# zeux/niagara

Measured on AMD Instinct MI355X. Metric: meshlets culled+compacted /sec, higher is better.
Workload: dtype f32; 1 GPU; config3A: 10000000 meshlets/GPU, 156250 task commands over 15625 draws, cone+frustum clustercull (LATE=0) + ordered compaction; meshlets_total=10000000, meshlets_rank0=10000000, commands_rank0=156250, draws_rank0=15625, streams=1, scatter_waves_per_workgroup=16, regime=one pass after the other on one stream, input_copies_rotated=4, count_reset=fused (NV_OPT_FUSED_COUNT_RESET), meshlet_layout=SoA12, visible_rank0=257819, visible_total=257819, counts_allreduce=none (N=1)

## Files before the change

niagara_amd/csrc/args.h:

```cpp
#pragma once

#include <hip/hip_runtime.h>
#include <stdint.h>

#include "../../include/niagara_vis.h"
#include "dealing.h"

#ifdef NV_EXPERIMENTS
#define NV_DBG(args, bits) (((args).debugMode & (bits)) != 0)
#else
#define NV_DBG(args, bits) false
#endif

namespace nv
{

#if defined(__HIP_DEVICE_COMPILE__) && !defined(__GFX9__)
#error "args.h: the DPP scans are written for GFX9-family wave64 targets (gfx950)"
#endif
#ifdef NV_EXPERIMENTS
#define NV_ASSERT_FULL_EXEC() do { if (__builtin_amdgcn_read_exec() != ~0ull) __builtin_trap(); } while (0)
#else
#define NV_ASSERT_FULL_EXEC() do { } while (0)
#endif

template <int CTRL, int ROW_MASK>
__device__ __forceinline__ uint32_t dpp_pull_u32(uint32_t v)
{
	return (uint32_t)__builtin_amdgcn_update_dpp(0, (int)v, CTRL, ROW_MASK, 0xf, false);
}

__device__ __forceinline__ uint32_t wave_scan_inclusive_u32(uint32_t v)
{
	NV_ASSERT_FULL_EXEC();
	v += dpp_pull_u32<0x111, 0xf>(v);
	v += dpp_pull_u32<0x112, 0xf>(v);
	v += dpp_pull_u32<0x114, 0xf>(v);
	v += dpp_pull_u32<0x118, 0xf>(v);
	v += dpp_pull_u32<0x142, 0xa>(v);
	v += dpp_pull_u32<0x143, 0xc>(v);
	return v;
}

template <int CTRL>
__device__ __forceinline__ uint32_t dpp_move_u32(uint32_t v)
{
	return (uint32_t)__builtin_amdgcn_update_dpp((int)v, (int)v, CTRL, 0xf, 0xf, false);
}
__device__ __forceinline__ uint32_t wave_shift_up1_u32(uint32_t v) { return dpp_move_u32<0x138>(v); }
__device__ __forceinline__ uint32_t quad_first_u32(uint32_t v) { return dpp_move_u32<0x00>(v); }
__device__ __forceinline__ uint32_t quad_xor1_u32(uint32_t v) { return dpp_move_u32<0xB1>(v); }
__device__ __forceinline__ uint32_t quad_xor2_u32(uint32_t v) { return dpp_move_u32<0x4E>(v); }

__device__ __forceinline__ uint32_t wave_sum_u32(uint32_t v)
{
	return (uint32_t)__builtin_amdgcn_readlane((int)wave_scan_inclusive_u32(v), 63);
}

constexpr uint32_t CC_MAX_SCATTER_TILES = 512;
constexpr uint32_t CC_COUNT_STRIDE = 16;
constexpr uint32_t CC_LISTS = 256;
struct ClusterCounts
{
	uint32_t parity;
	uint32_t k2parity;
	uint32_t base;
	uint32_t pad[29];
	uint32_t listOverflow[2];
	uint32_t pad2[30];
	uint32_t listCount[2][CC_LISTS * CC_COUNT_STRIDE];
	uint32_t counts[2][CC_MAX_SCATTER_TILES * CC_COUNT_STRIDE];
};

typedef __attribute__((address_space(4))) const uint32_t* nv_uniform_u32p;
__device__ __forceinline__ uint32_t load_uniform_u32(const uint32_t* p)
{
	return *(nv_uniform_u32p)(uintptr_t)p;
}

struct ClusterArgs
{
	NvCullData cd;
	NvPyramidDesc pyr;
	const NvMeshTaskCommand* __restrict__ commands;
	const uint32_t* __restrict__ count4;
	const NvMeshDraw* __restrict__ draws;
	const NvMeshlet* __restrict__ meshlets;
	const uint2* __restrict__ soaBounds;
	const uint32_t* __restrict__ soaCones;
	const float* __restrict__ poolBounds;
	const uint4* __restrict__ blockBounds;
	uint32_t blockMeshlets;
	uint32_t* __restrict__ mvb;
	uint32_t* __restrict__ clusterIndices;
	uint32_t* __restrict__ clusterCount4;
	uint32_t* __restrict__ payloadCounts;
	uint64_t* __restrict__ masks;
	uint4* __restrict__ candList;
	uint32_t listStride;
	uint32_t listMinPer;
	ClusterCounts* __restrict__ tileCounts;
	uint32_t scatterTiles;
	uint32_t generations;
	uint32_t dealScale;
	uint32_t cullWavesMagic;
	uint32_t genBlocks, genBlocksMagic;
	uint32_t tilesMagic;
	DealPlan plan;
	float filterK;
	float viewRowNorm;
	float viewTransNorm;
	float viewSum;
	uint32_t* hostHint;
	uint32_t commandCountOverride;
	float* __restrict__ probeOut;
#ifdef NV_EXPERIMENTS
	uint32_t debugMode;
#endif
	uint32_t fusedReset;
	uint32_t fusedSubmit;
	uint32_t deferHiz;
	uint32_t packBits;
	uint32_t packDirect;
	unsigned long long* countsSink;
};

struct DrawArgs
{
	NvCullData cd;
	NvPyramidDesc pyr;
	const NvMeshDraw* draws;
	const float4* __restrict__ soaWorld;
	const uint2* __restrict__ soaScaleMesh;
	const uint32_t* __restrict__ soaPostPass;
	const NvMesh* meshes;
	void* commands;
	uint32_t* count4;
	uint32_t* dvb;
	uint8_t* results;
	ClusterCounts* tileCounts;
	uint32_t scatterTiles;
	uint32_t fusedReset;
	uint32_t fusedSubmit;
	uint32_t meshCount;
	uint32_t* hostHint;
	uint32_t taskList;
	uint4* records;
	uint32_t* recordCounts;
	uint32_t recordsOn;
	uint32_t tileDraws;
	uint32_t unitsPerWave;
	uint32_t visFirst;
#ifdef NV_EXPERIMENTS
	uint32_t debugMode;
#endif
};

struct TriangleArgs
{
	NvGlobals globals;
	const NvMeshTaskCommand* __restrict__ commands;
	const NvMeshDraw* __restrict__ draws;
	const NvMeshlet* __restrict__ meshlets;
	const uint32_t* __restrict__ meshletData;
	const NvVertex* __restrict__ vertices;
	const uint32_t* __restrict__ clusterIndices;
	const uint32_t* __restrict__ cc4;
	NvTriangleMask* __restrict__ masks;
	uint32_t capacity;
	unsigned long long* __restrict__ totals;
	unsigned long long* __restrict__ partials;
};

struct RasterArgs
{
	NvGlobals globals;
	const NvMeshTaskCommand* __restrict__ commands;
	const NvMeshDraw* __restrict__ draws;
	const NvMeshlet* __restrict__ meshlets;
	const uint32_t* __restrict__ meshletData;
// ... 35 lines not shown
```

niagara_amd/csrc/clustercull.hip:

```cpp
#include <type_traits>

#include "cullmath.h"
#include "args.h"
#include "filtermath.h"
#include "dealing.h"
#include "cullform.h"

namespace nv
{

constexpr int CC_WAVES = 4;
constexpr int CC_THREADS = CC_WAVES * 64;


struct LaneData
{
	uint32_t b0, b1, cone;
	uint32_t mvbWord;
};

struct DrawUniform
{
	f3 q;
	float qw;
// ... 770 lines not shown
}

template <bool LATE, bool SOA, bool BITS, int CC_DA, bool DIRECT = false, bool DEFER = false, bool PACK = false>
__global__ __launch_bounds__(CC_THREADS, 6) void cluster_mask_kernel(ClusterArgs a)
{
	static_assert(!PACK || (DIRECT && SOA && !LATE), "the packed walk is a form of the direct early pass");
	const uint32_t lane = threadIdx.x & 63u;
	const uint32_t wave = __builtin_amdgcn_readfirstlane(threadIdx.x >> 6);
	const uint32_t w = blockIdx.x * CC_WAVES + wave;

	__shared__ float4 s_tab[PACK ? CC_WAVES : 1][PACK ? 64 : 1][CP_ENTRY / 16];
	__shared__ uint64_t s_heads[PACK ? CC_WAVES : 1][PACK ? CP_WINDOWS : 1];
	__shared__ uint64_t s_nout[PACK && !BITS ? CC_WAVES : 1][PACK && !BITS ? CP_WINDOWS : 1];

	__shared__ uint32_t s_mipTable[CC_WAVES][NV_MAX_MIPS];
	const uint32_t* s_mipOffset = s_mipTable[wave];
	if (LATE)
	{
		uint32_t off = 0;
#pragma unroll
		for (uint32_t i = 0; i < NV_MAX_MIPS; ++i)
			off = lane == i ? a.pyr.mipOffset[i] : off;
		if (lane < NV_MAX_MIPS)
			s_mipTable[wave][lane] = off;
	}

	if (!NV_DBG(a, 262144u))
		__builtin_amdgcn_s_setprio(3);
	const uint32_t gen = a.genBlocks ? div_launch_constant(blockIdx.x, a.genBlocks, a.genBlocksMagic) : 0u;
	float poolVmax3 = __builtin_inff(), poolRmax = __builtin_inff();
	uint32_t rawGroups, bankWord;
#ifdef NV_PLAIN_LOADS
	bankWord = load_uniform_u32(&a.tileCounts->parity);
	rawGroups = load_uniform_u32(a.count4 + 1);
	if (SOA)
	{
		k_f32p pb = (k_f32p)(uintptr_t)a.poolBounds;
		poolVmax3 = pb[0];
		poolRmax = pb[1];
	}
#else
	if (SOA)
	{
		uint64_t pool;
		asm volatile("s_nop 4\n\ts_load_dword %0, %3, 0x4\n\ts_load_dword %1, %4, 0x0\n\ts_load_dwordx2 %2, %5, 0x0\n\ts_waitcnt lgkmcnt(0)"
		             : "=&s"(rawGroups), "=&s"(bankWord), "=&s"(pool)
		             : "s"(a.count4), "s"(&a.tileCounts->parity), "s"(a.poolBounds)
		             : "memory");
		poolVmax3 = __uint_as_float((uint32_t)pool);
		poolRmax = __uint_as_float((uint32_t)(pool >> 32));
	}
	else
		asm volatile("s_nop 4\n\ts_load_dword %0, %2, 0x4\n\ts_load_dword %1, %3, 0x0\n\ts_waitcnt lgkmcnt(0)"
		             : "=&s"(rawGroups), "=&s"(bankWord)
		             : "s"(a.count4), "s"(&a.tileCounts->parity)
		             : "memory");
#endif
	const uint32_t numCmds = a.commandCountOverride ? a.commandCountOverride : (rawGroups < 65535u ? rawGroups : 65535u) * 64u;
	const uint32_t bank = bankWord & 1u;
	if (a.hostHint && blockIdx.x == 0 && threadIdx.x == 0)
		__hip_atomic_store(a.hostHint + (a.payloadCounts ? 4 : 0), numCmds, __ATOMIC_RELAXED, __HIP_MEMORY_SCOPE_SYSTEM);
	constexpr uint32_t CH = LATE ? CC_CHUNK_LATE : CC_CHUNK;
	const bool weightedWanted = !LATE && !NV_DBG(a, 32768u);
	const uint32_t planFlags = (weightedWanted ? DEAL_WEIGHTED_WANTED : 0u) | CH << 8;
	uint32_t chunkOf, myChunks, tileMul31, numTiles, gridWaves;
	bool dealtWeighted;
	{
		DealPlan plan;
		if (numCmds == a.plan.cmds && planFlags == a.plan.flags && !NV_DBG(a, 1073741824u))
			plan = a.plan;
		else
			plan = deal_plan(numCmds, CH, weightedWanted, gridDim.x * CC_WAVES, a.cullWavesMagic, a.generations, a.genBlocks, gridDim.x, a.dealScale, a.scatterTiles, a.tilesMagic);
		myChunks = deal_wave(plan, w, lane, gen, a.genBlocks * CC_WAVES, &chunkOf);
		gridWaves = plan.waves;
		dealtWeighted = plan.weighted != 0;
		tileMul31 = plan.tileMul31;
		numTiles = plan.numTiles;
	}
	const uint32_t myCmds = myChunks * CH;
	if (w == 0 && lane == 0)
	{
		a.tileCounts->k2parity = bank;
		a.tileCounts->base = a.fusedReset ? 0u : a.clusterCount4[0];
	}

	const bool dbgTime = NV_DBG(a, 8u) && a.probeOut;
	unsigned long long* stamps = reinterpret_cast<unsigned long long*>(a.probeOut) + (size_t)w * 8;
#define NV_STAMP(i) do { if (dbgTime && lane == 0) stamps[i] = __builtin_readcyclecounter(); } while (0)
	NV_STAMP(0);
	if (dbgTime && lane == 0)
		stamps[6] = wall_clock64();

	uint32_t passedFilter = 0;
#if defined(NV_FILLER_PS)
#pragma unroll
	for (int f = 0; f < NV_FILLER_PS; ++f)
		asm volatile("s_cmp_eq_u32 0, 0" : : : "scc");
#endif
#if defined(NV_FILLER_PV)
#pragma unroll
	for (int f = 0; f < NV_FILLER_PV; ++f)
		asm volatile("v_nop");
#endif
	for (uint32_t seg = 0; seg < myCmds; seg += 64)
	{
		const uint32_t cnt = myCmds - seg < 64u ? myCmds - seg : 64u;

		const uint32_t cidx = (seg + lane) / CH;
		const uint32_t chunk = dealtWeighted ? segment_chunk(chunkOf, seg >> 6) : cidx * gridWaves + w;
		const uint32_t myIdx = chunk * CH + (seg + lane) % CH;
		SegmentRegs r = {};
		if (lane < cnt && myIdx < numCmds)
		{
			const uint32_t* p = reinterpret_cast<const uint32_t*>(a.commands + myIdx);
			r.drawId = p[0];
			r.taskOffset = p[1];
			r.taskCount = p[2] < 64u ? p[2] : 64u;
			r.lateDrawVisibility = p[3];
			r.meshletVisibilityOffset = p[4];
		}
		if (!SOA)
		{
			if (r.taskCount)
			{
				const float4* d = reinterpret_cast<const float4*>(a.draws + r.drawId);
				r.d0 = d[0];
				r.d1 = d[1];
			}
			r.f = make_filter(a.cd, lane_draw(r), a.filterK, a.viewRowNorm, a.viewTransNorm, a.viewSum, poolVmax3, poolRmax);
		}
		NV_STAMP(1);

		constexpr bool FOLD_A = !LATE;
		constexpr bool BLOCK = SOA && !LATE && !BITS && !DIRECT && !DEFER;
		const bool foldSound = !FOLD_A || filter_fold_sound(a.cd.frustum);
		const bool useFilter = a.filterK > 0.0f && foldSound && !NV_DBG(a, 32u);
		u32x4 g0 = {}, g1 = {};
		auto gather_issue = [&]()
		{
			const char* dp = reinterpret_cast<const char*>(a.draws + (r.taskCount ? r.drawId : 0u));
#ifdef NV_PLAIN_LOADS
			g0 = reinterpret_cast<const u32x4*>(dp)[0];
			g1 = reinterpret_cast<const u32x4*>(dp)[1];
#else
			asm volatile("global_load_dwordx4 %0, %2, off\n\tglobal_load_dwordx4 %1, %2, off offset:16" : "=&v"(g0), "=&v"(g1) : "v"(dp) : "memory");
#endif
		};
		auto gather_finish = [&]()
		{
			r.d0 = make_float4(__uint_as_float(g0.x), __uint_as_float(g0.y), __uint_as_float(g0.z), __uint_as_float(g0.w));
			r.d1 = make_float4(__uint_as_float(g1.x), __uint_as_float(g1.y), __uint_as_float(g1.z), __uint_as_float(g1.w));
			r.f = make_filter<false>(a.cd, lane_draw(r), a.filterK, a.viewRowNorm, a.viewTransNorm, a.viewSum, poolVmax3, poolRmax);
			if (FOLD_A && !DIRECT)
			{
#pragma unroll
				for (int i = 0; i < 3; ++i)
				{
					r.fold[i] = a.cd.frustum[0] * r.f.m[i];
					r.fold[4 + i] = a.cd.frustum[2] * r.f.m[3 + i];
				}
				r.fold[3] = a.cd.frustum[0] * r.f.b[0];
				r.fold[7] = a.cd.frustum[2] * r.f.b[1];
			}
			if (!useFilter && !DIRECT)
				r.f.tK = __builtin_inff();
		};
// ... 467 lines not shown
			{
				const uint32_t n = (uint32_t)__builtin_popcountll(has);
				const uint32_t sub = w & (CC_LISTS - 1u);
				uint32_t slot = 0;
				if (lane == 0)
					slot = atomicAdd(&a.tileCounts->listCount[bank][sub * CC_COUNT_STRIDE], n);
				slot = __builtin_amdgcn_readfirstlane(slot);
				if (slot + n <= a.listStride)
				{
					if (has >> lane & 1ull)
					{
						uint4* e = a.candList + (size_t)(sub * a.listStride + slot + __builtin_amdgcn_mbcnt_hi((uint32_t)(has >> 32), __builtin_amdgcn_mbcnt_lo((uint32_t)has, 0u))) * 2u;
						e[0] = make_uint4(myIdx, r.drawId, r.taskOffset, r.taskCount);
						e[1] = make_uint4(r.lateDrawVisibility, r.meshletVisibilityOffset, maskLo, maskHi);
					}
				}
				else if (lane == 0)
					atomicOr(&a.tileCounts->listOverflow[bank], 1u);
			}
		}
		if (lane < cnt && myIdx < numCmds)
		{
			const uint64_t m = ((uint64_t)maskHi << 32) | maskLo;
			a.masks[myIdx] = m;
		}
		const bool payloadForm = !LATE && !DEFER && a.payloadCounts != nullptr;
		if (payloadForm)
		{
			const bool liveCmd = lane < cnt && myIdx < numCmds;
			const uint32_t mlo = liveCmd ? maskLo : 0u, mhi = liveCmd ? maskHi : 0u;
			if (liveCmd)
				a.payloadCounts[myIdx] = (uint32_t)__builtin_popcount(mlo) + (uint32_t)__builtin_popcount(mhi);
			for (uint64_t owners = __ballot((mlo | mhi) != 0); owners; owners &= owners - 1)
			{
				const uint32_t src = (uint32_t)__builtin_ctzll(owners);
				const uint32_t lo = __builtin_amdgcn_readlane(mlo, src), hi = __builtin_amdgcn_readlane(mhi, src);
				const uint32_t ci = __builtin_amdgcn_readlane(myIdx, src);
				if ((lane < 32u ? lo >> lane : hi >> (lane - 32u)) & 1u)
					a.clusterIndices[(size_t)ci * 64 + __builtin_amdgcn_mbcnt_hi(hi, __builtin_amdgcn_mbcnt_lo(lo, 0u))] = ci | (lane << 24);
			}
		}
		{
			const bool live = lane < cnt && myIdx < numCmds;
			const uint64_t m = live ? ((uint64_t)maskHi << 32) | maskLo : 0ull;
			const uint32_t tileOf = live ? deal_tile_of(myIdx, tileMul31) : ~0u;
			uint32_t pc = (uint32_t)__builtin_popcountll(m);
			const uint32_t tile0 = quad_first_u32(tileOf);
			const bool quadUniform = __all_quad_same(tileOf, tile0);
			if (quadUniform)
			{
				pc += quad_xor1_u32(pc);
				pc += quad_xor2_u32(pc);
				if (lane & 3u)
					pc = 0;
			}
			if (pc && !DEFER && !payloadForm && !NV_DBG(a, 2048u))
				atomicAdd(&a.tileCounts->counts[bank][tileOf * CC_COUNT_STRIDE], pc);
		}
	}
	if (lane == 0 && passedFilter && !(!LATE && !DEFER && a.payloadCounts != nullptr))
	{
		const uint32_t spread = numTiles ? (1u << (31 - __builtin_clz(numTiles))) - 1u : 0u;
		atomicAdd(&a.tileCounts->counts[bank][(w & spread) * CC_COUNT_STRIDE + 1], passedFilter);
	}
	NV_STAMP(5);
	if (dbgTime && lane == 0)
		stamps[7] = wall_clock64();
#undef NV_STAMP
}

template <int SC_WAVES>
__global__ __launch_bounds__(SC_WAVES * 64) void cluster_scatter_kernel(ClusterArgs a)
{
	constexpr uint32_t SC_THREADS = SC_WAVES * 64;
	__shared__ uint32_t s_part[SC_WAVES];
	__shared__ uint32_t s_sum[SC_WAVES];
	constexpr uint32_t STEP = 1024, PER_LANE = STEP / SC_THREADS;
	constexpr int TILE_LOADS = (int)((CC_MAX_SCATTER_TILES + SC_THREADS - 1) / SC_THREADS);

	const uint32_t tid = threadIdx.x;
	const uint32_t lane = tid & 63u;
	const uint32_t wave = __builtin_amdgcn_readfirstlane(tid >> 6);

	const uint32_t numCmds = indirect_command_count(a);
	const uint32_t T = scatter_tile_commands(numCmds, a.scatterTiles, a.tilesMagic);
	const uint32_t numTiles = (numCmds + T - 1) / T;
	const uint32_t tile = blockIdx.x;
	const bool dbgNoScatter = NV_DBG(a, 4u);

	const uint32_t k2parity = load_uniform_u32(&a.tileCounts->k2parity);
	const uint32_t base0 = load_uniform_u32(&a.tileCounts->base);
	uint32_t cnt0[TILE_LOADS] = {}, cnt1[TILE_LOADS] = {};
	uint32_t pf0[TILE_LOADS] = {}, pf1[TILE_LOADS] = {};
#pragma unroll
	for (int j = 0; j < TILE_LOADS; ++j)
	{
		const uint32_t i = j * SC_THREADS + tid;
		if (i < numTiles)
		{
			cnt0[j] = a.tileCounts->counts[0][i * CC_COUNT_STRIDE];
			cnt1[j] = a.tileCounts->counts[1][i * CC_COUNT_STRIDE];
			pf0[j] = a.tileCounts->counts[0][i * CC_COUNT_STRIDE + 1];
			pf1[j] = a.tileCounts->counts[1][i * CC_COUNT_STRIDE + 1];
		}
	}
	const uint32_t first = tile * T;
	const uint32_t n = tile < numTiles ? (numCmds - first < T ? numCmds - first : T) : 0u;
	uint64_t m4[PER_LANE];
	if (PER_LANE == 4)
	{
		const uint32_t c = tid * PER_LANE;
		const ulonglong2* src = reinterpret_cast<const ulonglong2*>(a.masks + first + c);
		ulonglong2 lo = make_ulonglong2(0, 0), hi = make_ulonglong2(0, 0);
		if (c < n)
		{
			lo = src[0];
			hi = src[1];
		}
		m4[0] = c + 0 < n ? lo.x : 0ull;
		m4[PER_LANE > 1 ? 1 : 0] = c + 1 < n ? lo.y : 0ull;
		m4[PER_LANE > 2 ? 2 : 0] = c + 2 < n ? hi.x : 0ull;
		m4[PER_LANE > 3 ? 3 : 0] = c + 3 < n ? hi.y : 0ull;
	}
	else
	{
#pragma unroll
		for (uint32_t j = 0; j < PER_LANE; ++j)
			m4[j] = tid * PER_LANE + j < n ? a.masks[first + tid * PER_LANE + j] : 0ull;
	}

	const uint32_t bank = k2parity & 1u;
	for (uint32_t i = tile * SC_THREADS + tid; i < CC_MAX_SCATTER_TILES; i += gridDim.x * SC_THREADS)
	{
		a.tileCounts->counts[bank ^ 1u][i * CC_COUNT_STRIDE] = 0;
		a.tileCounts->counts[bank ^ 1u][i * CC_COUNT_STRIDE + 1] = 0;
		if (i < CC_LISTS)
			a.tileCounts->listCount[bank ^ 1u][i * CC_COUNT_STRIDE] = 0;
	}
	if (tile == 0 && tid == 0)
	{
		a.tileCounts->parity = bank ^ 1u;
		a.tileCounts->listOverflow[bank ^ 1u] = 0;
		if (numTiles == 0 && a.hostHint)
			__hip_atomic_store(a.hostHint + 1, 0u, __ATOMIC_RELAXED, __HIP_MEMORY_SCOPE_SYSTEM);
		if (numTiles == 0)
		{
			if (a.fusedReset)
				a.clusterCount4[0] = 0;
			if (a.countsSink)
			{
				a.countsSink[0] = 0;
				a.countsSink[1] = a.count4[0];
				a.countsSink[2] = a.fusedReset ? 0u : a.clusterCount4[0];
			}
			if (a.fusedSubmit)
			{
				const uint32_t raw = a.fusedReset ? 0u : a.clusterCount4[0];
				const uint32_t count = raw < NV_CLUSTER_LIMIT ? raw : NV_CLUSTER_LIMIT;
				const uint32_t gy = (count + 255u) / 256u;
				a.clusterCount4[1] = NV_CLUSTER_TILE;
				a.clusterCount4[2] = gy < 65535u ? gy : 65535u;
				a.clusterCount4[3] = 256u / NV_CLUSTER_TILE;
				for (uint32_t i = count; i < ((count + 255u) & ~255u); ++i)
					a.clusterIndices[i] = ~0u;
			}
		}
	}
	if (tile >= numTiles)
		return;

	uint32_t before = 0, all = 0, passed = 0;
#pragma unroll
	for (int j = 0; j < TILE_LOADS; ++j)
	{
		const uint32_t i = j * SC_THREADS + tid;
		const uint32_t v = bank ? cnt1[j] : cnt0[j];
		all += v;
		before += i < tile ? v : 0u;
		passed += bank ? pf1[j] : pf0[j];
	}
	if (tile == numTiles - 1 && a.hostHint)
	{
		__shared__ uint32_t s_passed;
		if (tid == 0)
			s_passed = 0;
		__syncthreads();
		const uint32_t wp = wave_sum_u32(passed);
		if (lane == 0 && wp)
			atomicAdd(&s_passed, wp);
		__syncthreads();
		if (tid == 0)
			__hip_atomic_store(a.hostHint + 1, s_passed, __ATOMIC_RELAXED, __HIP_MEMORY_SCOPE_SYSTEM);
	}
	const uint32_t wBefore = wave_sum_u32(before), wAll = wave_sum_u32(all);
	if (lane == 0)
	{
		s_part[wave] = wBefore;
		s_sum[wave] = wAll;
	}
	__syncthreads();
	uint32_t running = base0, total = base0;
#pragma unroll
	for (int w = 0; w < SC_WAVES; ++w)
	{
		running += s_part[w];
		total += s_sum[w];
	}
	if (tid == 0 && tile == numTiles - 1)
	{
		a.clusterCount4[0] = total;
		if (a.countsSink)
		{
			a.countsSink[0] = 0;
			a.countsSink[1] = a.count4[0];
			a.countsSink[2] = total;
		}
	}
	if (a.fusedSubmit && tile == numTiles - 1)
	{
		const uint32_t count = total < NV_CLUSTER_LIMIT ? total : NV_CLUSTER_LIMIT;
		if (tid == 0)
		{
			const uint32_t gy = (count + 255u) / 256u;
			a.clusterCount4[1] = NV_CLUSTER_TILE;
			a.clusterCount4[2] = gy < 65535u ? gy : 65535u;
			a.clusterCount4[3] = 256u / NV_CLUSTER_TILE;
		}
		const uint32_t boundary = (count + 255u) & ~255u;
		if (count + tid < boundary)
			a.clusterIndices[count + tid] = ~0u;
	}

	for (uint32_t c0 = 0; c0 < n; c0 += STEP)
	{
		if (c0)
		{
			const uint32_t c = c0 + tid * PER_LANE;
#pragma unroll
			for (uint32_t j = 0; j < PER_LANE; ++j)
				m4[j] = c + j < n ? a.masks[first + c + j] : 0ull;
		}
		uint32_t pc[PER_LANE], mine = 0;
#pragma unroll
		for (uint32_t j = 0; j < PER_LANE; ++j)
		{
			pc[j] = (uint32_t)__builtin_popcountll(m4[j]);
			mine += pc[j];
		}
		uint32_t incl = wave_scan_inclusive_u32(mine);
		__syncthreads();
		if (lane == 63)
			s_part[wave] = incl;
		__syncthreads();
		uint32_t excl = running + incl - mine;
#pragma unroll
		for (int w = 0; w < SC_WAVES; ++w)
		{
			uint32_t p = s_part[w];
			excl += w < (int)wave ? p : 0u;
			running += p;
		}

		const bool mayOverflow = running > NV_CLUSTER_LIMIT;
		auto emit = [&](auto checked)
		{
#pragma unroll
			for (uint32_t j = 0; j < PER_LANE; ++j)
			{
				uint64_t owners = dbgNoScatter ? 0ull : __ballot(pc[j] != 0);
				while (owners)
				{
					const int src = __builtin_ctzll(owners);
					asm("s_bitset0_b64 %0, %1" : "+s"(owners) : "s"(src));
					const uint32_t mlo = __builtin_amdgcn_readlane((uint32_t)m4[j], src);
					const uint32_t mhi = __builtin_amdgcn_readlane((uint32_t)(m4[j] >> 32), src);
					const uint32_t off = __builtin_amdgcn_readlane(excl, src);
					const uint64_t ms = ((uint64_t)mhi << 32) | mlo;
					if (ms >> lane & 1ull)
					{
						uint32_t rank = __builtin_amdgcn_mbcnt_hi(mhi, __builtin_amdgcn_mbcnt_lo(mlo, 0u));
						uint32_t index = off + rank;
						if (!decltype(checked)::value || index < NV_CLUSTER_LIMIT)
							a.clusterIndices[index] = (first + c0 + (wave * 64 + src) * PER_LANE + j) | (lane << 24);
					}
				}
				excl += pc[j];
			}
		};
		if (mayOverflow)
			emit(std::true_type{});
		else
			emit(std::false_type{});
	}
}

constexpr int CH_THREADS = 256;
constexpr int CH_CMDS = 128;
#ifndef NV_CH_U
#define NV_CH_U 4
#endif
constexpr int CH_U = NV_CH_U;

#define NV_LDS_BARRIER() asm volatile("s_waitcnt lgkmcnt(0)\n\ts_barrier" ::: "memory")

struct HizTimes
{
	bool on;
	uint64_t prev;
	uint64_t acc[6];
	uint32_t rounds;
};
#ifdef NV_EXPERIMENTS
#define NV_HIZ_T(T, i, drain)                                                  \
	do                                                                         \
	{                                                                          \
		if ((T).on)                                                            \
		{                                                                      \
			if (drain)                                                         \
				asm volatile("s_waitcnt vmcnt(0) lgkmcnt(0)" ::: "memory");    \
			const uint64_t now = __builtin_readcyclecounter();                 \
			(T).acc[i] += now - (T).prev;                                      \
			(T).prev = now;                                                    \
		}                                                                      \
	} while (0)
#else
#define NV_HIZ_T(T, i, drain) do { } while (0)
#endif

template <int U, bool SOA, bool FIRST>
NV_DEV void hiz_round(const ClusterArgs& a, uint32_t base, uint32_t total, uint32_t tid, bool ownsDraw, const float4& d0, const float4& d1,
                      const uint16_t* s_list, const uint32_t* s_taskOffset, float4 (*s_draw)[2], const MipRecord* s_mip, uint32_t* s_visLo, uint32_t* s_visHi,
                      HizTimes& T)
{
	const float* __restrict__ texels = a.pyr.d_base;
	uint32_t e[U];
	uint2 b[U];
#pragma unroll
	for (int k = 0; k < U; ++k)
	{
		const uint32_t s = base + k * CH_THREADS + tid;
		e[k] = s_list[s < total ? s : total - 1u];
		const uint32_t mi = s_taskOffset[e[k] >> 6] + (e[k] & 63u);
		if (SOA)
			b[k] = a.soaBounds[mi];
		else
			b[k] = *reinterpret_cast<const uint2*>(a.meshlets + mi);
	}
	if (FIRST)
	{
		if (ownsDraw)
		{
			s_draw[tid][0] = d0;
			s_draw[tid][1] = d1;
		}
		NV_LDS_BARRIER();
	}
	NV_HIZ_T(T, 1, true);
	float depth[U];
	uint32_t use[U];
	float t00[U], t10[U], t01[U], t11[U];
#pragma unroll
	for (int k = 0; k < U; ++k)
	{
		const float4 q0 = s_draw[e[k] >> 6][0], q1 = s_draw[e[k] >> 6][1];
		DrawUniform u;
		u.pos = { q0.x, q0.y, q0.z };
		u.scale = q0.w;
		u.q = { q1.x, q1.y, q1.z };
		u.qw = q1.w;
		LaneData l;
		l.b0 = b[k].x;
		l.b1 = b[k].y;
		l.cone = 0;
		l.mvbWord = 0;
		f3 c;
// ... 356 lines not shown
			const float len = __builtin_amdgcn_sqrtf(__builtin_fmaf(cx, cx, __builtin_fmaf(cy, cy, cz * cz)));
			const float rhs = __builtin_fmaf(kc * 0.00787401574803149606f, len, scale * rad);
			const float D = lhs - rhs;
			const bool cull = D > Tc, keep = D < -Tc;
			decided = decided && (out || cull || keep);
			visible = visible && keep;
		}
		if (!decided && !NV_DBG(a, 536870912u))
		{
			const float4 q0 = s_draw[owner][0], q1 = s_draw[owner][1];
			DrawUniform u;
			u.pos = { q0.x, q0.y, q0.z };
			u.scale = q0.w;
			u.q = { q1.x, q1.y, q1.z };
			u.qw = q1.w;
			LaneData l;
			l.b0 = b0;
			l.b1 = b1;
			l.cone = cone[k];
			l.mvbWord = 0;
			f3 c;
			float r;
			lane_sphere(cd, u, l, c, r);
			visible = frustum_test(cd, c, r);
			if (cd.clusterBackfaceEnabled != 0 && visible)
			{
				f3 axis;
				float cutoff;
				lane_cone(cd, u, l, axis, cutoff);
				visible = !cone_cull(c, r, axis, cutoff);
			}
		}
		if (STAT)
		{
			const bool passes = s < total && !(useCert && out);
			const uint64_t passM = __ballot(passes);
			const uint32_t lane = tid & 63u;
			const uint32_t prevOwner = wave_shift_up1_u32(owner);
			if (passes && (lane == 0u || prevOwner != owner || !(passM >> (lane - 1u) & 1ull)))
				s_passed[owner] = 1u;
		}
		if (s < total && !visible)
			atomicAnd(bit < 32u ? &s_visLo[owner] : &s_visHi[owner], ~(1u << (bit & 31u)));
	}
}

struct BitsCommand
{
	uint32_t drawId, taskOffset, taskCount, mvo;
};

NV_DEV BitsCommand bits_load_command(const ClusterArgs& a, uint32_t idx, bool live)
{
	const uint32_t* p = reinterpret_cast<const uint32_t*>(a.commands + (live ? idx : 0u));
	BitsCommand c;
	c.drawId = p[0];
	c.taskOffset = p[1];
	c.taskCount = p[2] < 64u ? p[2] : 64u;
	c.mvo = p[4];
	return c;
}

template <bool SOA, bool BITS>
__global__ __launch_bounds__(CB_THREADS, 4) void cluster_bits_kernel(ClusterArgs a)
{
	__shared__ uint32_t s_visLo[CB_CMDS], s_visHi[CB_CMDS], s_taskOffset[CB_CMDS], s_excl[CB_CMDS], s_passed[BITS ? 1 : CB_CMDS];
	__shared__ float4 s_draw[CB_CMDS][2];
	__shared__ float4 s_cert[CB_CMDS][5];
	__shared__ uint16_t s_list[CB_CMDS * 64];
	__shared__ uint32_t s_part[CB_THREADS / 64];

	const uint32_t tid = threadIdx.x;
	const uint32_t lane = tid & 63u;
	const uint32_t wave = __builtin_amdgcn_readfirstlane(tid >> 6);
	const uint32_t numCmds = indirect_command_count(a);
	if (a.hostHint && blockIdx.x == 0 && tid == 0)
		__hip_atomic_store(a.hostHint + (a.payloadCounts ? 4 : 0), numCmds, __ATOMIC_RELAXED, __HIP_MEMORY_SCOPE_SYSTEM);
	const uint32_t T2 = scatter_tile_commands(numCmds, a.scatterTiles, a.tilesMagic);
	const uint32_t bank = load_uniform_u32(&a.tileCounts->parity) & 1u;
	if (blockIdx.x == 0 && tid == 0)
	{
		a.tileCounts->k2parity = bank;
		a.tileCounts->base = a.fusedReset ? 0u : a.clusterCount4[0];
	}
	if (numCmds == 0)
		return;
	const uint32_t G = gridDim.x;
	const uint32_t iters = (numCmds + G * (uint32_t)CB_CMDS - 1u) / (G * (uint32_t)CB_CMDS);
	uint32_t per = iters ? (numCmds + G * iters - 1u) / (G * iters) : 0u;
	per = per < 16u ? 16u : per;
	uint32_t passedAcc = 0;

	uint32_t chunk = blockIdx.x;
	BitsCommand cur = bits_load_command(a, chunk * per + tid, tid < per && chunk * per + tid < numCmds);
	BitsCommand nxt = bits_load_command(a, (chunk + G) * per + tid, tid < per && (chunk + G) * per + tid < numCmds);
	float4 d0, d1;
	uint32_t oldw[3];
	auto load_dependents = [&](const BitsCommand& c, bool liveC, float4& o0, float4& o1, uint32_t* w)
	{
		const uint32_t tc = liveC ? c.taskCount : 0u;
		const float4* dp = reinterpret_cast<const float4*>(a.draws + (tc ? c.drawId : 0u));
		o0 = dp[0];
		o1 = dp[1];
		const uint32_t w0 = tc ? c.mvo >> 5 : 0u, wLast = tc ? (c.mvo + tc - 1u) >> 5 : 0u;
#pragma unroll
		for (uint32_t j = 0; j < 3; ++j)
			w[j] = BITS ? a.mvb[w0 + j < wLast ? w0 + j : wLast] : 0u;
	};
	load_dependents(cur, tid < per && chunk * per + tid < numCmds, d0, d1, oldw);
	asm volatile("; prologue loads landed" : "+v"(d0.x), "+v"(d0.y), "+v"(d0.z), "+v"(d0.w), "+v"(d1.x), "+v"(d1.y), "+v"(d1.z), "+v"(d1.w), "+v"(oldw[0]), "+v"(oldw[1]), "+v"(oldw[2]),
	             "+v"(nxt.drawId), "+v"(nxt.taskOffset), "+v"(nxt.taskCount), "+v"(nxt.mvo));

	for (; chunk * per < numCmds; chunk += G)
	{
		const uint32_t idx = chunk * per + tid;
		const bool live = tid < per && idx < numCmds;
		const uint32_t taskCount = live ? cur.taskCount : 0u;
		uint64_t cand = 0;
		{
			const uint32_t sh = cur.mvo & 31u;
			uint64_t old = 0;
#pragma unroll
			for (int j = 0; j < 3; ++j)
			{
				const int lo = 32 * j - (int)sh;
				if (lo >= (int)taskCount)
					break;
				old |= lo >= 0 ? (uint64_t)oldw[j] << lo : (uint64_t)(oldw[j] >> (-lo));
			}
			const uint64_t valid = taskCount >= 64u ? ~0ull : (1ull << taskCount) - 1ull;
			cand = BITS ? old & valid : valid;
		}

		const uint32_t pc = (uint32_t)__builtin_popcountll(cand);
		uint32_t incl = wave_scan_inclusive_u32(pc);
		if (lane == 63)
			s_part[wave] = incl;
		if (tid < CB_CMDS)
		{
			s_visLo[tid] = (uint32_t)cand;
			s_visHi[tid] = (uint32_t)(cand >> 32);
			s_taskOffset[tid] = cur.taskOffset;
			s_excl[tid] = incl - pc;
			if (!BITS)
				s_passed[tid] = 0u;
		}

		const float4 c0 = d0, c1 = d1;
		float4 n0, n1;
		uint32_t neww[3];
		load_dependents(nxt, tid < per && idx + G * per < numCmds, n0, n1, neww);
		const uint32_t idx2 = (chunk + 2u * G) * per + tid;
		const BitsCommand nn = bits_load_command(a, idx2, tid < per && idx2 < numCmds);
		NV_LDS_BARRIER();

		uint32_t total = 0;
		{
			const uint32_t p0 = s_part[0], p1 = s_part[1];
			total = p0 + p1;
			if (NV_DBG(a, 67108864u))
			{
				uint32_t at = tid < (uint32_t)CB_CMDS ? s_excl[tid] + (tid >= 64u ? p0 : 0u) : 0u;
				for (uint64_t rest = cand; rest; rest &= rest - 1)
					s_list[at++] = (uint16_t)((tid << 6) | (uint32_t)__builtin_ctzll(rest));
			}
			else
// ... 364 lines not shown
```

niagara_amd/csrc/context.hip:

```cpp
#include <hip/hip_runtime.h>

#include <atomic>
#include <new>
#include <algorithm>
#include <vector>
#include <stdlib.h>
#include <stdint.h>
#include <string.h>
#include <math.h>

#include "../../include/niagara_vis.h"
#include "cullmath.h"
#include "args.h"
#include "filtermath.h"
#include "cullform.h"

namespace nv
{

int launch_cluster_mask(hipStream_t, const ClusterArgs&, const CullForm&, uint32_t maskBlocks);
int launch_cluster_scatter(hipStream_t, const ClusterArgs&, uint32_t scatterBlocks, uint32_t waves);
int launch_cluster_hiz(hipStream_t, const ClusterArgs&, bool soa, uint32_t gridBlocks);
int launch_cluster_bits(hipStream_t, const ClusterArgs&, bool soa, uint32_t gridBlocks);
size_t clustercull_mask_bytes();
// ... 804 lines not shown

	if (nv::drawcull_result_bytes(cull->drawCount) > ctx->drawResultsCapacity)
		return NV_ENOMEM;
	int rc = NV_OK;

	nv::DrawArgs a;
	a.cd = *cull;
	a.pyr = pyramid ? *pyramid : null_pyramid();
	a.draws = d_draws;
	const size_t drawOffset = ctx->scene->drawsFrom && d_draws >= ctx->scene->drawsFrom ? (size_t)(d_draws - ctx->scene->drawsFrom) : ~size_t(0);
	const bool mirrored = ctx->scene->soaWorld && drawOffset != ~size_t(0) && ctx->scene->drawsFrom + drawOffset == d_draws &&
	                      drawOffset + cull->drawCount <= ctx->scene->drawsCount && ctx->scene->drawsMeshes == d_meshes;
	a.soaWorld = mirrored ? ctx->scene->soaWorld + drawOffset : nullptr;
	a.soaScaleMesh = mirrored ? ctx->scene->soaScaleMesh + drawOffset : nullptr;
	a.soaPostPass = mirrored ? ctx->scene->soaPostPass + drawOffset : nullptr;
	a.meshes = d_meshes;
	a.commands = d_commands;
	a.count4 = d_count4;
	a.dvb = d_drawVisibility;
	a.results = ctx->drawResults;
	a.tileCounts = ctx->drawTileCounts;
	a.scatterTiles = scatter_grid(ctx);
#ifdef NV_EXPERIMENTS
	a.debugMode = ctx->debugMode;
#endif
	a.fusedReset = ctx->fusedReset;
	a.fusedSubmit = ctx->fusedSubmit;
	a.meshCount = ctx->scene->meshesFrom == d_meshes ? ctx->scene->meshCount : 0u;
	a.hostHint = ctx->hintDevice;
	a.taskList = ctx->forceTaskList >= 0 ? (uint32_t)ctx->forceTaskList : (ctx->hintHost && ctx->hintHost[3] > 4u * ctx->hintHost[2] ? 1u : 0u);
	a.visFirst = late ? 0u : (ctx->forceVisFirst >= 0 ? (uint32_t)ctx->forceVisFirst : (ctx->hintHost && ctx->hintHost[2] != 0u && (uint64_t)ctx->hintHost[2] * 8u < cull->drawCount ? 1u : 0u));
	if (task)
	{
		ctx->variants[a.taskList ? NV_VARIANT_TASK_LIST : NV_VARIANT_TASK_PER_DRAW] += 1u;
		ctx->taskCommandsFrom = d_commands;
	}
	hipEvent_t e0 = prof_mark(ctx, (hipStream_t)stream);
	rc = nv::launch_drawcull((hipStream_t)stream, a, late, task);
	prof_push(ctx, NV_PROF_DRAWCULL, e0, prof_mark(ctx, (hipStream_t)stream));
	return rc;
}

int nv_reset_count(nv_context* ctx, void* stream, uint32_t* d_count4a, uint32_t* d_count4b)
{
	if (!ctx || (!d_count4a && !d_count4b))
		return NV_EINVAL;
	DeviceGuard guard(ctx->device);
	return nv::launch_reset_count((hipStream_t)stream, d_count4a, d_count4b);
}

int nv_tasksubmit(nv_context* ctx, void* stream, uint32_t* d_count4, NvMeshTaskCommand* d_commands)
{
	if (!ctx || !d_count4 || !d_commands)
		return NV_EINVAL;
	DeviceGuard guard(ctx->device);
	return nv::launch_tasksubmit((hipStream_t)stream, d_count4, d_commands);
}

static int fill_cluster_args(nv_context* ctx, nv::ClusterArgs& a, const NvCullData* cull, int late,
                             const NvMeshTaskCommand* d_commands, const uint32_t* d_count4, const NvMeshDraw* d_draws,
                             const NvMeshlet* d_meshlets, uint32_t* d_meshletVisibility, const NvPyramidDesc* pyramid)
{
	if (!ctx || !cull || !d_commands || !d_draws || !d_meshlets)
		return NV_EINVAL;
	if (cull->clusterOcclusionEnabled == 1 && !d_meshletVisibility)
		return NV_EINVAL;
	if (late && cull->clusterOcclusionEnabled == 1 && !(pyramid && pyramid->d_base))
		return NV_EINVAL;
	memset(&a, 0, sizeof(a));
	a.cd = *cull;
	a.pyr = pyramid ? *pyramid : null_pyramid();
	a.commands = d_commands;
	a.count4 = d_count4;
	a.draws = d_draws;
	a.meshlets = d_meshlets;
	const bool soa = ctx->scene->mirroredFrom == d_meshlets && ctx->scene->soaBounds && ctx->scene->poolWords;
	a.soaBounds = soa ? ctx->scene->soaBounds : nullptr;
	a.soaCones = soa ? ctx->scene->soaCones : nullptr;
	a.poolBounds = soa ? reinterpret_cast<const float*>(ctx->scene->poolWords + 2) : nullptr;
	a.blockBounds = soa ? ctx->scene->blockBounds : nullptr;
	a.blockMeshlets = soa ? ctx->scene->mirroredCount : 0u;
	a.mvb = d_meshletVisibility;
	a.masks = ctx->masks;
	a.candList = ctx->candList;
	a.listStride = ctx->listStride;
	a.listMinPer = ctx->listMinPer;
	a.tileCounts = ctx->tileCounts;
	a.scatterTiles = scatter_grid(ctx);
	a.generations = ctx->ccBlocksPerCU;
	a.dealScale = ctx->dealScale;
	{
		const uint32_t cullGrid = persistent_grid(ctx, ctx->ccBlocksPerCU);
		a.cullWavesMagic = nv_division_magic(cullGrid * 4u);
		a.genBlocks = cullGrid / 6u ? cullGrid / 6u : 1u;
		a.genBlocksMagic = nv_division_magic(a.genBlocks);
		a.tilesMagic = nv_division_magic(a.scatterTiles);
	}
	a.filterK = nv::filter_k(cull->frustum, cull->znear, cull->zfar);
	nv::filter_view_norms(cull->view, &a.viewRowNorm, &a.viewTransNorm, &a.viewSum);
	a.hostHint = ctx->hintDevice;
	return NV_OK;
}

int nv_clustercull(nv_context* ctx, void* stream, const NvCullData* cull, int late, const NvMeshTaskCommand* d_commands,
                   const uint32_t* d_count4, const NvMeshDraw* d_draws, const NvMeshlet* d_meshlets,
                   uint32_t* d_meshletVisibility, const NvPyramidDesc* pyramid, uint32_t* d_clusterIndices,
                   uint32_t* d_clusterCount4)
{
	if (!d_count4 || !d_clusterIndices || !d_clusterCount4)
		return NV_EINVAL;
	nv::ClusterArgs a;
	int rc = fill_cluster_args(ctx, a, cull, late, d_commands, d_count4, d_draws, d_meshlets, d_meshletVisibility, pyramid);
	if (rc)
		return rc;
	DeviceGuard guard(ctx->device);
	a.clusterIndices = d_clusterIndices;
	a.clusterCount4 = d_clusterCount4;
	a.fusedReset = ctx->fusedReset;
	a.fusedSubmit = ctx->fusedSubmit;
	a.countsSink = reinterpret_cast<unsigned long long*>(ctx->countsSink);
#ifdef NV_EXPERIMENTS
	a.debugMode = ctx->debugMode;
	if (ctx->debugMode & (8u | 268435456u))
	{
		const size_t timingWaves = std::max((size_t)persistent_grid(ctx, 8) * 4, (size_t)ctx->listSharers * nv::CC_LISTS * 4);
		if (ctx->timing && ctx->timingWaves < timingWaves)
		{
			scratch_free(ctx->timing);
			ctx->timing = nullptr;
		}
		if (!ctx->timing && scratch_alloc(&ctx->timing, timingWaves * 8 * sizeof(unsigned long long)) == hipSuccess)
			ctx->timingWaves = timingWaves;
		a.probeOut = ctx->timing;
	}
#endif
	hipStream_t s = (hipStream_t)stream;
	hipEvent_t e0 = prof_mark(ctx, s);
	const bool twoStage = launch_cull(ctx, s, a, false, late, d_commands, &rc).twoStage;
	ctx->variants[NV_VARIANT_HIZ_STAGE] += twoStage ? 1u : 0u;
	hipEvent_t e1 = prof_mark(ctx, s);
	hipEvent_t eh = e1;
	if (rc == 0 && twoStage)
	{
		const uint32_t blocks = ctx->listSharers * nv::CC_LISTS;
		rc = nv::launch_cluster_hiz(s, a, a.soaBounds != nullptr, blocks);
		eh = prof_mark(ctx, s);
	}
	if (rc == 0 && !(ctx->debugMode & 16u))
		rc = nv::launch_cluster_scatter(s, a, a.scatterTiles, ctx->scatterWaves);
	hipEvent_t e2 = prof_mark(ctx, s);
	prof_push(ctx, NV_PROF_CLUSTER_CULL, e0, e1);
	if (twoStage)
		prof_push(ctx, NV_PROF_CLUSTER_HIZ, e1 ? e1 : nullptr, eh);
	prof_push(ctx, NV_PROF_CLUSTER_SCATTER, eh ? eh : nullptr, e2);
	return rc;
}

int nv_clustersubmit(nv_context* ctx, void* stream, uint32_t* d_clusterCount4, uint32_t* d_clusterIndices)
{
	if (!ctx || !d_clusterCount4 || !d_clusterIndices)
		return NV_EINVAL;
	DeviceGuard guard(ctx->device);
	return nv::launch_clustersubmit((hipStream_t)stream, d_clusterCount4, d_clusterIndices);
}

int nv_taskcull(nv_context* ctx, void* stream, const NvCullData* cull, int late, const NvMeshTaskCommand* d_commands,
                const uint32_t* d_count4, const NvMeshDraw* d_draws, const NvMeshlet* d_meshlets,
                uint32_t* d_meshletVisibility, const NvPyramidDesc* pyramid, uint32_t* d_payloads, uint32_t* d_payloadCounts)
{
	if (!d_count4 || !d_payloads || !d_payloadCounts)
		return NV_EINVAL;
	nv::ClusterArgs a;
	int rc = fill_cluster_args(ctx, a, cull, late, d_commands, d_count4, d_draws, d_meshlets, d_meshletVisibility, pyramid);
	if (rc)
		return rc;
	DeviceGuard guard(ctx->device);
	a.clusterIndices = d_payloads;
	a.payloadCounts = d_payloadCounts;
	if (!late && !ctx->taskcullOneLaunch)
	{
		a.fusedReset = 1u;
		a.clusterCount4 = nullptr;
		(void)launch_cull(ctx, (hipStream_t)stream, a, true, 0, d_commands, &rc);
		return rc;
	}
	return nv::launch_taskcull((hipStream_t)stream, a, late, a.soaBounds != nullptr, (uint32_t)ctx->numCUs * 8);
}

int nv_cluster_expand(nv_context* ctx, void* stream, const NvMeshTaskCommand* d_commands, const NvMeshlet* d_meshlets,
                      const uint32_t* d_clusterIndices, const uint32_t* d_clusterCount4, NvClusterRecord* d_records,
                      uint32_t recordCapacity, uint64_t* d_totals3)
{
	if (!ctx || !d_commands || !d_meshlets || !d_clusterIndices || !d_clusterCount4 || !d_totals3 || (!d_records && recordCapacity))
		return NV_EINVAL;
	DeviceGuard guard(ctx->device);
	const uint32_t grid = persistent_grid(ctx, 8);
	return nv::launch_cluster_expand((hipStream_t)stream, d_commands, d_meshlets, d_clusterIndices, d_clusterCount4, d_records, recordCapacity,
	                                 d_totals3, ctx->totalsPartials, grid);
}

int nv_trianglecull(nv_context* ctx, void* stream, const NvGlobals* globals, const NvMeshTaskCommand* d_commands, const NvMeshDraw* d_draws,
                    const NvMeshlet* d_meshlets, const uint32_t* d_meshletData, const NvVertex* d_vertices, const uint32_t* d_clusterIndices,
                    const uint32_t* d_clusterCount4, NvTriangleMask* d_masks, uint32_t maskCapacity, uint64_t* d_totals3)
{
	if (!ctx || !globals || !d_commands || !d_draws || !d_meshlets || !d_meshletData || !d_vertices || !d_clusterIndices || !d_clusterCount4 ||
	    !d_totals3 || (!d_masks && maskCapacity))
		return NV_EINVAL;
	DeviceGuard guard(ctx->device);
	nv::TriangleArgs a;
	a.globals = *globals;
	a.commands = d_commands;
	a.draws = d_draws;
	a.meshlets = d_meshlets;
	a.meshletData = d_meshletData;
	a.vertices = d_vertices;
	a.clusterIndices = d_clusterIndices;
	a.cc4 = d_clusterCount4;
	a.masks = d_masks;
	a.capacity = maskCapacity;
	a.totals = reinterpret_cast<unsigned long long*>(d_totals3);
	const uint32_t grid = persistent_grid(ctx, 8);
// ... 330 lines not shown
```

Measured before the change: 525.7 billion meshlets/s.

## Speculatively load scatter masks using host-predicted command count before counts arrive

After: 513.5 billion meshlets/s. 2.3% lower.

```diff
diff --git a/niagara_amd/csrc/args.h b/niagara_amd/csrc/args.h
--- a/niagara_amd/csrc/args.h
+++ b/niagara_amd/csrc/args.h
@@ -1,10 +1,12 @@
 #pragma once
 
 #include <hip/hip_runtime.h>
+#include <stddef.h>
 #include <stdint.h>
 
 #include "../../include/niagara_vis.h"
 #include "dealing.h"
+#include "scatterspan.h"
 
 #ifdef NV_EXPERIMENTS
 #define NV_DBG(args, bits) (((args).debugMode & (bits)) != 0)
@@ -65,7 +67,8 @@
 	uint32_t parity;
 	uint32_t k2parity;
 	uint32_t base;
-	uint32_t pad[29];
+	uint32_t cmds;
+	uint32_t pad[28];
 	uint32_t listOverflow[2];
 	uint32_t pad2[30];
 	uint32_t listCount[2][CC_LISTS * CC_COUNT_STRIDE];
@@ -77,6 +80,11 @@
 {
 	return *(nv_uniform_u32p)(uintptr_t)p;
 }
+__device__ __forceinline__ uint32_t load_uniform_pinned_u32(const uint32_t* p)
+{
+	return *(volatile nv_uniform_u32p)(uintptr_t)p;
+}
+static_assert(offsetof(ClusterCounts, cmds) == 12 && offsetof(ClusterCounts, listOverflow) == 128, "ClusterCounts: drawcull.hip shares the layout");
 
 struct ClusterArgs
 {
@@ -96,6 +104,7 @@
 	uint32_t* __restrict__ clusterCount4;
 	uint32_t* __restrict__ payloadCounts;
 	uint64_t* __restrict__ masks;
+	uint32_t maskCmds;
 	uint4* __restrict__ candList;
 	uint32_t listStride;
 	uint32_t listMinPer;
diff --git a/niagara_amd/csrc/clustercull.hip b/niagara_amd/csrc/clustercull.hip
--- a/niagara_amd/csrc/clustercull.hip
+++ b/niagara_amd/csrc/clustercull.hip
@@ -876,6 +876,7 @@
 	{
 		a.tileCounts->k2parity = bank;
 		a.tileCounts->base = a.fusedReset ? 0u : a.clusterCount4[0];
+		a.tileCounts->cmds = numCmds;
 	}
 
 	const bool dbgTime = NV_DBG(a, 8u) && a.probeOut;
@@ -1509,52 +1510,63 @@
 	const uint32_t lane = tid & 63u;
 	const uint32_t wave = __builtin_amdgcn_readfirstlane(tid >> 6);
 
-	const uint32_t numCmds = indirect_command_count(a);
-	const uint32_t T = scatter_tile_commands(numCmds, a.scatterTiles, a.tilesMagic);
-	const uint32_t numTiles = (numCmds + T - 1) / T;
 	const uint32_t tile = blockIdx.x;
 	const bool dbgNoScatter = NV_DBG(a, 4u);
 
-	const uint32_t k2parity = load_uniform_u32(&a.tileCounts->k2parity);
-	const uint32_t base0 = load_uniform_u32(&a.tileCounts->base);
+	const uint32_t guessCmds = a.commandCountOverride ? a.commandCountOverride : a.plan.cmds;
+	const ScatterSpan guess = scatter_span(guessCmds, tile, a.scatterTiles, a.tilesMagic);
+	uint32_t specOffset = scatter_spec_first(guess, a.maskCmds) + tid * PER_LANE, specCount = guess.n;
+	constexpr uint32_t BANK_WORDS = CC_MAX_SCATTER_TILES * CC_COUNT_STRIDE;
+	asm volatile("" : "+v"(specOffset), "+v"(specCount) : "s"(a.masks), "s"(a.tileCounts));
+	uint32_t k2parity = load_uniform_pinned_u32(&a.tileCounts->k2parity), base0 = load_uniform_pinned_u32(&a.tileCounts->base),
+	         numCmds = load_uniform_pinned_u32(&a.tileCounts->cmds);
+	const uint64_t* specSrc = a.masks + specOffset;
+	const uint32_t* countSrc = &a.tileCounts->counts[0][tid * CC_COUNT_STRIDE];
 	uint32_t cnt0[TILE_LOADS] = {}, cnt1[TILE_LOADS] = {};
 	uint32_t pf0[TILE_LOADS] = {}, pf1[TILE_LOADS] = {};
 #pragma unroll
 	for (int j = 0; j < TILE_LOADS; ++j)
 	{
 		const uint32_t i = j * SC_THREADS + tid;
-		if (i < numTiles)
-		{
-			cnt0[j] = a.tileCounts->counts[0][i * CC_COUNT_STRIDE];
-			cnt1[j] = a.tileCounts->counts[1][i * CC_COUNT_STRIDE];
-			pf0[j] = a.tileCounts->counts[0][i * CC_COUNT_STRIDE + 1];
-			pf1[j] = a.tileCounts->counts[1][i * CC_COUNT_STRIDE + 1];
-		}
-	}
-	const uint32_t first = tile * T;
-	const uint32_t n = tile < numTiles ? (numCmds - first < T ? numCmds - first : T) : 0u;
+		if (i < CC_MAX_SCATTER_TILES)
+		{
+			cnt0[j] = countSrc[j * SC_THREADS * CC_COUNT_STRIDE];
+			cnt1[j] = countSrc[j * SC_THREADS * CC_COUNT_STRIDE + BANK_WORDS];
+			pf0[j] = countSrc[j * SC_THREADS * CC_COUNT_STRIDE + 1];
+			pf1[j] = countSrc[j * SC_THREADS * CC_COUNT_STRIDE + BANK_WORDS + 1];
+		}
+	}
 	uint64_t m4[PER_LANE];
-	if (PER_LANE == 4)
-	{
-		const uint32_t c = tid * PER_LANE;
-		const ulonglong2* src = reinterpret_cast<const ulonglong2*>(a.masks + first + c);
-		ulonglong2 lo = make_ulonglong2(0, 0), hi = make_ulonglong2(0, 0);
-		if (c < n)
-		{
-			lo = src[0];
-			hi = src[1];
-		}
-		m4[0] = c + 0 < n ? lo.x : 0ull;
-		m4[PER_LANE > 1 ? 1 : 0] = c + 1 < n ? lo.y : 0ull;
-		m4[PER_LANE > 2 ? 2 : 0] = c + 2 < n ? hi.x : 0ull;
-		m4[PER_LANE > 3 ? 3 : 0] = c + 3 < n ? hi.y : 0ull;
-	}
-	else
-	{
-#pragma unroll
-		for (uint32_t j = 0; j < PER_LANE; ++j)
-			m4[j] = tid * PER_LANE + j < n ? a.masks[first + tid * PER_LANE + j] : 0ull;
-	}
+	auto load_first_step = [&](const uint64_t* mine, uint32_t count)
+	{
+		if (PER_LANE == 4)
+		{
+			const uint32_t c = tid * PER_LANE;
+			const ulonglong2* src = reinterpret_cast<const ulonglong2*>(mine);
+			ulonglong2 lo = make_ulonglong2(0, 0), hi = make_ulonglong2(0, 0);
+			if (c < count)
+			{
+				lo = src[0];
+				hi = src[1];
+			}
+			m4[0] = c + 0 < count ? lo.x : 0ull;
+			m4[PER_LANE > 1 ? 1 : 0] = c + 1 < count ? lo.y : 0ull;
+			m4[PER_LANE > 2 ? 2 : 0] = c + 2 < count ? hi.x : 0ull;
+			m4[PER_LANE > 3 ? 3 : 0] = c + 3 < count ? hi.y : 0ull;
+		}
+		else
+		{
+#pragma unroll
+			for (uint32_t j = 0; j < PER_LANE; ++j)
+				m4[j] = tid * PER_LANE + j < count ? mine[j] : 0ull;
+		}
+	};
+	load_first_step(specSrc, specCount);
+	asm volatile("" : "+s"(k2parity), "+s"(base0), "+s"(numCmds));
+	const ScatterSpan span = scatter_span(numCmds, tile, a.scatterTiles, a.tilesMagic);
+	const uint32_t numTiles = span.numTiles, first = span.first, n = span.n;
+	if (!scatter_spec_accepted(guess, span, a.maskCmds))
+		load_first_step(a.masks + first + tid * PER_LANE, n);
 
 	const uint32_t bank = k2parity & 1u;
 	for (uint32_t i = tile * SC_THREADS + tid; i < CC_MAX_SCATTER_TILES; i += gridDim.x * SC_THREADS)
@@ -1605,19 +1617,6 @@
 		all += v;
 		before += i < tile ? v : 0u;
 		passed += bank ? pf1[j] : pf0[j];
-	}
-	if (tile == numTiles - 1 && a.hostHint)
-	{
-		__shared__ uint32_t s_passed;
-		if (tid == 0)
-			s_passed = 0;
-		__syncthreads();
-		const uint32_t wp = wave_sum_u32(passed);
-		if (lane == 0 && wp)
-			atomicAdd(&s_passed, wp);
-		__syncthreads();
-		if (tid == 0)
-			__hip_atomic_store(a.hostHint + 1, s_passed, __ATOMIC_RELAXED, __HIP_MEMORY_SCOPE_SYSTEM);
 	}
 	const uint32_t wBefore = wave_sum_u32(before), wAll = wave_sum_u32(all);
 	if (lane == 0)
@@ -1718,6 +1717,20 @@
 			emit(std::true_type{});
 		else
 			emit(std::false_type{});
+	}
+
+	if (tile == numTiles - 1 && a.hostHint)
+	{
+		__shared__ uint32_t s_passed;
+		if (tid == 0)
+			s_passed = 0;
+		__syncthreads();
+		const uint32_t wp = wave_sum_u32(passed);
+		if (lane == 0 && wp)
+			atomicAdd(&s_passed, wp);
+		__syncthreads();
+		if (tid == 0)
+			__hip_atomic_store(a.hostHint + 1, s_passed, __ATOMIC_RELAXED, __HIP_MEMORY_SCOPE_SYSTEM);
 	}
 }
 
@@ -2240,6 +2253,7 @@
 	{
 		a.tileCounts->k2parity = bank;
 		a.tileCounts->base = a.fusedReset ? 0u : a.clusterCount4[0];
+		a.tileCounts->cmds = numCmds;
 	}
 	if (numCmds == 0)
 		return;
diff --git a/niagara_amd/csrc/context.hip b/niagara_amd/csrc/context.hip
--- a/niagara_amd/csrc/context.hip
+++ b/niagara_amd/csrc/context.hip
@@ -910,6 +910,7 @@
 	a.blockMeshlets = soa ? ctx->scene->mirroredCount : 0u;
 	a.mvb = d_meshletVisibility;
 	a.masks = ctx->masks;
+	a.maskCmds = (uint32_t)(nv::clustercull_mask_bytes() / sizeof(uint64_t));
 	a.candList = ctx->candList;
 	a.listStride = ctx->listStride;
 	a.listMinPer = ctx->listMinPer;
@@ -964,7 +965,9 @@
 #endif
 	hipStream_t s = (hipStream_t)stream;
 	hipEvent_t e0 = prof_mark(ctx, s);
-	const bool twoStage = launch_cull(ctx, s, a, false, late, d_commands, &rc).twoStage;
+	const nv::CullForm form = launch_cull(ctx, s, a, false, late, d_commands, &rc);
+	const bool twoStage = form.twoStage;
+	a.plan.cmds = form.expectedCmds;
 	ctx->variants[NV_VARIANT_HIZ_STAGE] += twoStage ? 1u : 0u;
 	hipEvent_t e1 = prof_mark(ctx, s);
 	hipEvent_t eh = e1;
diff --git a/niagara_amd/csrc/scatterspan.h b/niagara_amd/csrc/scatterspan.h
--- /dev/null
+++ b/niagara_amd/csrc/scatterspan.h
@@ -0,0 +1,41 @@
+#pragma once
+
+#include <stdint.h>
+
+#include "dealing.h"
+
+namespace nv
+{
+
+constexpr uint32_t SCATTER_STEP = 1024;
+
+struct ScatterSpan
+{
+	uint32_t T;
+	uint32_t numTiles;
+	uint32_t first;
+	uint32_t n;
+};
+
+NV_DP ScatterSpan scatter_span(uint32_t numCmds, uint32_t tile, uint32_t tiles, uint32_t tilesMagic)
+{
+	ScatterSpan s;
+	s.T = deal_tile_commands(numCmds, tiles, tilesMagic);
+	s.numTiles = (numCmds + s.T - 1u) / s.T;
+	s.first = tile * s.T;
+	s.n = tile < s.numTiles ? (numCmds - s.first < s.T ? numCmds - s.first : s.T) : 0u;
+	return s;
+}
+
+NV_DP uint32_t scatter_spec_first(const ScatterSpan& guess, uint32_t scratchCmds)
+{
+	const uint32_t last = (scratchCmds - SCATTER_STEP) & ~1u;
+	return guess.first < last ? guess.first : last;
+}
+
+NV_DP bool scatter_spec_accepted(const ScatterSpan& guess, const ScatterSpan& truth, uint32_t scratchCmds)
+{
+	return guess.T == truth.T && guess.first == truth.first && guess.n == truth.n && scatter_spec_first(guess, scratchCmds) == truth.first;
+}
+
+}
```
